# ltatzel/PyTorchHessianFree

Hardware: AMD Instinct MI355X
Metric: GGN-matvecs/sec (damped operator calls inside the PCG loop) (higher is better)
Workload: dtype f32

## Files before the change

### pytorchhessianfree_amd/csrc/hf_conv.hip

```cpp

#include <hip/hip_runtime.h>
#include <stdint.h>
#include <stdlib.h>
#include <string.h>

#include "hf_pcg.h"
#include "hf_unpack.h"

namespace {

typedef float f32x16 __attribute__((ext_vector_type(16)));

constexpr int CT = 256;
#ifndef HF_CONV_BK
#define HF_CONV_BK 32
#endif
constexpr int MAX_TAPS = 64;
#ifndef HF_CONV_FLAT96
#define HF_CONV_FLAT96 1
#endif
#ifndef HF_DCLASS_NOSPLIT
#define HF_DCLASS_NOSPLIT 1
#endif
#ifndef HF_FLAT96_MIN_WORK
#define HF_FLAT96_MIN_WORK 2048
#endif

template <int WM_, int WN_, int TM_, int TN_, int BK_>
struct Cfg {
  static constexpr int WM = WM_, WN = WN_, TM = TM_, TN = TN_, BK = BK_;
  static constexpr int BM = 32 * WM * TM, BN = 32 * WN * TN;
  static constexpr int SM = (BM + 63) / 64 * 64, SN = (BN + 63) / 64 * 64;
  static constexpr int KQ = BK / 4;
  static constexpr int RPT = CT / KQ;
  static constexpr int HK = BK / 2;
  static constexpr int LDK = BK + 4;
  static constexpr int LDA = SM + 4, LDB = SN + 4;
  static constexpr int NT_FLOATS = 2 * (SM + SN) * LDK;
  static constexpr int TN_FLOATS = 2 * BK * (LDA + LDB);
  static constexpr int LDS_FLOATS = (NT_FLOATS > TN_FLOATS ? NT_FLOATS : TN_FLOATS) + 4;
  static_assert(WM * WN == 4, "four waves");
  static_assert(SM / RPT == 2 && SN / RPT == 2, "the hand-counted prefetch ring assumes 2 + 2 loads per step (NT)");
  static_assert(SM == SN, "both operands are staged at the same width");
  static_assert(LDS_FLOATS * 4 <= 64 * 1024, "static LDS limit");
};
typedef Cfg<2, 2, 1, 1, HF_CONV_BK> Small;
typedef Cfg<2, 2, 2, 2, 16> Big;
typedef Cfg<4, 1, 1, 3, 16> Big96;
typedef Cfg<1, 4, 3, 1, 16> Flat96;

struct FastDiv {
  unsigned mul, shift;
};
__host__ __device__ __forceinline__ unsigned fdiv(unsigned n, FastDiv f) {
#if defined(__HIP_DEVICE_COMPILE__)
  return (__umulhi(n, f.mul) + n) >> f.shift;
#else
  return (unsigned)((((unsigned long long)n * f.mul) >> 32) + n) >> f.shift;
#endif
}

struct ConvArgs {
  const float* src;
  const float* mat;
  float* out;
  float* ws;
  int* tickets;
  int dgrad;
  int rows;
  int rh, rw;
  int sh_, sw_;
  int cs, cs_ld;
  int mat_ld;
  int nout, ldc;
  int kout;
  int R, S, stride_h, stride_w, pad_h, pad_w;
  int ntaps;
  int tap_rs[MAX_TAPS];
  int tiles_m, tiles_n, splits, steps;
  int scalar;
  int shift_h, shift_w;
  int out_c;
  int slabs;
  long long slab_stride;
  int big;
  int ncls;
  int cls_tile0[5];
  int cls_tap0[5];
  int cls_h[4], cls_w[4], cls_py[4], cls_px[4];
  FastDiv fd_tiles_n, fd_tiles_m, fd_splits, fd_rw, fd_rh, fd_csteps, fd_cblocks, fd_cs;
  const float *bn_x, *bn_mean, *bn_rstd;
  float *bn_part_x, *bn_part_1;
};

__device__ __forceinline__ void touch_args(const ConvArgs& a) {
  const int* ka = reinterpret_cast<const int*>(&a);
  int sink = 0;
#pragma unroll
  for (unsigned l = 0; l < (sizeof(ConvArgs) + 63) / 64; ++l) {
    const unsigned w = l * 16 < sizeof(ConvArgs) / 4 ? l * 16 : (unsigned)(sizeof(ConvArgs) / 4 - 1);
    sink ^= ka[w];
  }
  asm volatile("" ::"s"(sink));
}

__device__ __forceinline__ int gather_pixel(const ConvArgs& a, int n, int y, int x, int r, int q, bool& valid) {
  int sy, sx;
  bool v = true;
  if (!a.dgrad) {
    sy = y * a.stride_h - a.pad_h + r;
    sx = x * a.stride_w - a.pad_w + q;
  } else {
    const int ty = y + a.pad_h - r, tx = x + a.pad_w - q;
    if (a.shift_h >= 0) { sy = ty >> a.shift_h; sx = tx >> a.shift_w; }
    else { sy = ty / a.stride_h; sx = tx / a.stride_w; }
    v = (ty >= 0) & (tx >= 0) & (sy * a.stride_h == ty) & (sx * a.stride_w == tx);
  }
  v = v & ((unsigned)sy < (unsigned)a.sh_) & ((unsigned)sx < (unsigned)a.sw_);
  valid = v;
  return v ? (n * a.sh_ + sy) * a.sw_ + sx : 0;
}

__device__ __forceinline__ float4 ldg4(const float* p) { return *reinterpret_cast<const float4*>(p); }

typedef float f32x4 __attribute__((ext_vector_type(4)));
__device__ __forceinline__ void gload4(f32x4& dst, const float* p) {
  asm volatile("global_load_dwordx4 %0, %1, off" : "=v"(dst) : "v"(p) : "memory");
}
#define HF_WAIT_SLOT(N, A, B) \
  asm volatile("s_waitcnt vmcnt(" #N ")" : "+v"(A[0]), "+v"(A[1]), "+v"(B[0]), "+v"(B[1]) : : "memory")

__device__ __forceinline__ float4 ldg4s(const float* p, int valid) {
  float4 v = make_float4(0.f, 0.f, 0.f, 0.f);
  if (valid > 0) v.x = p[0];
  if (valid > 1) v.y = p[1];
  if (valid > 2) v.z = p[2];
  if (valid > 3) v.w = p[3];
  return v;
}

template <typename C, bool CLS = false, bool BNSUM = false>
__device__ __forceinline__ void finish_tile(const ConvArgs& a, const f32x16 (&acc)[C::TM][C::TN], int tile, int split,
                                            int wm, int wn, int lane, float* out_tile_base,
                                            int row0, int col0, int row_lim, int col_lim, int ldc,
                                            int* flag_lds, int cls = -1, float* lds = nullptr) {
  constexpr int BM = C::BM, BN = C::BN;
  const int i = lane & 31, h = lane >> 5;
  if constexpr (BNSUM) {
    static_assert(C::TM == 1 && C::TN == 1 && !CLS, "per-tile column sums: 64x64 tiles, plain row enumeration");
    const int col = wn * 32 + i, gcol = col0 + col;
    const bool cok = gcol < col_lim;
    const float mu = cok ? a.bn_mean[gcol] : 0.f, rs = cok ? a.bn_rstd[gcol] : 0.f;
    float xv[16];
#pragma unroll
    for (int reg = 0; reg < 16; ++reg) {
      const int orow = row0 + wm * 32 + (reg & 3) + 8 * (reg >> 2) + 4 * h;
      xv[reg] = (cok && orow < row_lim) ? a.bn_x[(size_t)orow * ldc + gcol] : mu;
    }
    double s1 = 0.0, sx = 0.0;
#pragma unroll
    for (int reg = 0; reg < 16; ++reg) {
      const int orow = row0 + wm * 32 + (reg & 3) + 8 * (reg >> 2) + 4 * h;
      if (cok && orow < row_lim) {
        const float v = acc[0][0][reg];
        s1 += (double)v;
        sx += (double)v * (double)(float)((xv[reg] - mu) * rs);
      }
    }
    double* red = reinterpret_cast<double*>(lds);
    red[(0 * 4 + wm * 2 + h) * BN + col] = s1;
    red[(1 * 4 + wm * 2 + h) * BN + col] = sx;
    __syncthreads();
    const int t = threadIdx.x;
    if (t < 2 * BN) {
      const int kind = t / BN, c = t - kind * BN;
      const double sum = ((red[(kind * 4 + 0) * BN + c] + red[(kind * 4 + 1) * BN + c]) +
                          red[(kind * 4 + 2) * BN + c]) + red[(kind * 4 + 3) * BN + c];
      const int tile_m = (int)fdiv((unsigned)tile, a.fd_tiles_n);
      if (col0 + c < col_lim)
        (kind ? a.bn_part_x : a.bn_part_1)[(size_t)(tile_m * a.splits + split) * a.nout + col0 + c] = (float)sum;
    }
  }
  if (a.splits == 1 || a.slabs) {
    float* dst = out_tile_base + (a.slabs ? (size_t)split * (size_t)a.slab_stride : 0);
#pragma unroll
    for (int im = 0; im < C::TM; ++im)
#pragma unroll
      for (int reg = 0; reg < 16; ++reg) {
        const int row = (wm * C::TM + im) * 32 + (reg & 3) + 8 * (reg >> 2) + 4 * h;
        int orow = row0 + row;
        bool rok = orow < row_lim;
        if (CLS && cls >= 0) {
          const int wc = a.cls_w[cls], hc = a.cls_h[cls];
          const int xq = orow % wc, tq = orow / wc;
          const int yq = tq % hc, nq = tq / hc;
          orow = (nq * a.rh + yq * a.stride_h + a.cls_py[cls]) * a.rw + xq * a.stride_w + a.cls_px[cls];
        }
#pragma unroll
        for (int in = 0; in < C::TN; ++in) {
          const int col = (wn * C::TN + in) * 32 + i;
          if (rok && col0 + col < col_lim) dst[(size_t)orow * ldc + col0 + col] = acc[im][in][reg];
        }
      }
    return;
  }
  const int tiles = a.tiles_m * a.tiles_n;
  float* mine = a.ws + ((size_t)split * tiles + tile) * (BM * BN);
#pragma unroll
  for (int im = 0; im < C::TM; ++im)
#pragma unroll
    for (int in = 0; in < C::TN; ++in)
#pragma unroll
      for (int reg = 0; reg < 16; ++reg) {
        const int row = (wm * C::TM + im) * 32 + (reg & 3) + 8 * (reg >> 2) + 4 * h;
        const int col = (wn * C::TN + in) * 32 + i;
        __hip_atomic_store(mine + row * BN + col, acc[im][in][reg], __ATOMIC_RELAXED, __HIP_MEMORY_SCOPE_AGENT);
      }
  asm volatile("s_waitcnt vmcnt(0)" ::: "memory");
  __syncthreads();
  if (threadIdx.x == 0) {
    const int old = __hip_atomic_fetch_add(a.tickets + tile, 1, __ATOMIC_RELAXED, __HIP_MEMORY_SCOPE_AGENT);
    const int last = old == a.splits - 1;
    if (last) {
      __hip_atomic_store(a.tickets + tile, 0, __ATOMIC_RELAXED, __HIP_MEMORY_SCOPE_AGENT);
      __builtin_amdgcn_fence(__ATOMIC_ACQUIRE, "agent");
      asm volatile("s_waitcnt vmcnt(0)" ::: "memory");
    }
    *flag_lds = last;
  }
  __syncthreads();
  if (!*flag_lds) return;
  const float* base = a.ws + (size_t)tile * (BM * BN);
  const size_t slab = (size_t)tiles * (BM * BN);
  for (int e = threadIdx.x; e < BM * BN / 4; e += CT) {
    float4 s = *reinterpret_cast<const float4*>(base + 4 * e);
    int sp = 1;
    for (; sp + 4 <= a.splits; sp += 4) {
      float4 v[4];
#pragma unroll
      for (int u = 0; u < 4; ++u) v[u] = *reinterpret_cast<const float4*>(base + (sp + u) * slab + 4 * e);
#pragma unroll
      for (int u = 0; u < 4; ++u) { s.x += v[u].x; s.y += v[u].y; s.z += v[u].z; s.w += v[u].w; }
    }
    for (; sp < a.splits; ++sp) {
      const float4 v = *reinterpret_cast<const float4*>(base + sp * slab + 4 * e);
      s.x += v.x; s.y += v.y; s.z += v.z; s.w += v.w;
    }
    const int row = (4 * e) / BN, col = (4 * e) % BN;
    if (row0 + row < row_lim) {
      float* o = out_tile_base + (size_t)(row0 + row) * ldc + col0 + col;
      const float v[4] = {s.x, s.y, s.z, s.w};
#pragma unroll
      for (int c = 0; c < 4; ++c)
        if (col0 + col + c < col_lim) o[c] = v[c];
    }
  }
}

template <bool SCALAR, typename C, bool CLS = false, bool BNSUM = false>
__device__ __forceinline__ void conv_nt_body(const ConvArgs& a, float* lds, int bid) {
  constexpr int BM = C::BM, BN = C::BN, BK = C::BK, KQ = C::KQ, RPT = C::RPT, HK = C::HK, LDK = C::LDK;
  constexpr int NU = 2;
  constexpr int SM = C::SM, SN = C::SN;
  float (*As)[SM][LDK] = reinterpret_cast<float (*)[SM][LDK]>(lds);
  float (*Bs)[SN][LDK] = reinterpret_cast<float (*)[SN][LDK]>(lds + 2 * SM * LDK);
  int& flag = *reinterpret_cast<int*>(lds + C::LDS_FLOATS - 4);
  touch_args(a);
  const int t = threadIdx.x, lane = t & 63, wave = t >> 6, wm = wave / C::WN, wn = wave % C::WN;
  const int bq = (int)fdiv((unsigned)bid, a.fd_tiles_n), tile_n = bid - bq * a.tiles_n;
  const int split = (int)fdiv((unsigned)bq, a.fd_tiles_m), tile_m = bq - split * a.tiles_m;
  const int tile = tile_m * a.tiles_n + tile_n;
  const int csteps = (a.cs + BK - 1) / BK;
  int cls = -1, row_base = tile_m * BM, rows_c = a.rows, tap0 = 0, steps = a.steps;
  if (CLS && a.ncls > 0) {
    cls = 0;
    while (cls + 1 < a.ncls && tile_m >= a.cls_tile0[cls + 1]) ++cls;
    row_base = (tile_m - a.cls_tile0[cls]) * BM;
    rows_c = (a.rows / (a.rh * a.rw)) * a.cls_h[cls] * a.cls_w[cls];
    tap0 = a.cls_tap0[cls];
    steps = (a.cls_tap0[cls + 1] - tap0) * csteps;
  }
  const int per = (int)fdiv((unsigned)(steps + a.splits - 1), a.fd_splits);
  const int j0 = split * per < steps ? split * per : steps, j1 = (j0 + per < steps) ? j0 + per : steps;

  const int lr = t / KQ, kq = t % KQ;
  int rn[NU], ry[NU], rx[NU];
#pragma unroll
  for (int u = 0; u < NU; ++u) {
    const int m = row_base + lr + RPT * u;
    if (m < rows_c) {
      if (CLS && cls >= 0) {
        const int wc = a.cls_w[cls], hc = a.cls_h[cls];
        const int xx = m % wc, tq = m / wc;
        rx[u] = xx * a.stride_w + a.cls_px[cls]; ry[u] = (tq % hc) * a.stride_h + a.cls_py[cls]; rn[u] = tq / hc;
      } else {
        const int tq = (int)fdiv((unsigned)m, a.fd_rw), xx = m - tq * a.rw;
        rn[u] = (int)fdiv((unsigned)tq, a.fd_rh);
        rx[u] = xx; ry[u] = tq - rn[u] * a.rh;
      }
    } else {
      rn[u] = -1; ry[u] = rx[u] = 0;
    }
  }
  const int RS = a.R * a.S;
  const float* brow[NU];
  bool bok[NU];
#pragma unroll
  for (int u = 0; u < NU; ++u) {
    const int j = tile_n * BN + lr + RPT * u;
    bok[u] = (j < a.nout) & (lr + RPT * u < BN);
    brow[u] = a.mat + (size_t)(bok[u] ? j : 0) * RS * a.mat_ld;
  }

  auto fetch = [&](int step, float4 (&ra)[NU], float4 (&rb)[NU]) -> unsigned {
    const int tl = step / csteps, c = (step - tl * csteps) * BK + 4 * kq, ti = tap0 + tl;
    const int rs_ = a.tap_rs[ti], r = rs_ & 255, q = rs_ >> 8;
    const bool cok = c < a.cs;
    unsigned ok = 0;
#pragma unroll
    for (int u = 0; u < NU; ++u) {
      bool va;
      const int pix = gather_pixel(a, rn[u], ry[u], rx[u], r, q, va);
      va = va & cok & (rn[u] >= 0);
      const bool vb = cok & bok[u];
      const float* pa = a.src + (va ? (size_t)pix * a.cs_ld + c : 0);
      const float* pb = vb ? brow[u] + (size_t)(r * a.S + q) * a.mat_ld + c : a.mat;
      ra[u] = ldg4s(pa, va ? a.cs - c : 0);
      rb[u] = ldg4s(pb, vb ? a.cs - c : 0);
      ok |= (va ? 1u : 0u) << (2 * u) | (vb ? 2u : 0u) << (2 * u);
    }
    return ok;
  };
  auto stash = [&](int buf, const float4 (&ra)[NU], const float4 (&rb)[NU], unsigned ok) {
    const float4 zero = make_float4(0.f, 0.f, 0.f, 0.f);
#pragma unroll
    for (int u = 0; u < NU; ++u) {
      *reinterpret_cast<float4*>(&As[buf][lr + RPT * u][4 * kq]) = (ok >> (2 * u)) & 1u ? ra[u] : zero;
      *reinterpret_cast<float4*>(&Bs[buf][lr + RPT * u][4 * kq]) = (ok >> (2 * u)) & 2u ? rb[u] : zero;
    }
  };

  f32x16 acc[C::TM][C::TN];
#pragma unroll
  for (int im = 0; im < C::TM; ++im)
#pragma unroll
    for (int in = 0; in < C::TN; ++in)
#pragma unroll
      for (int r = 0; r < 16; ++r) acc[im][in][r] = 0.f;
  const int i = lane & 31, h = lane >> 5;
  auto compute = [&](int cur) {
    float av[C::TM][HK], bv[C::TN][HK];
#pragma unroll
    for (int im = 0; im < C::TM; ++im) {
      const float* ap = &As[cur][(wm * C::TM + im) * 32 + i][HK * h];
#pragma unroll
      for (int v = 0; v < HK / 4; ++v)
        *reinterpret_cast<float4*>(av[im] + 4 * v) = *reinterpret_cast<const float4*>(ap + 4 * v);
    }
#pragma unroll
    for (int in = 0; in < C::TN; ++in) {
      const float* bp = &Bs[cur][(wn * C::TN + in) * 32 + i][HK * h];
#pragma unroll
      for (int v = 0; v < HK / 4; ++v)
        *reinterpret_cast<float4*>(bv[in] + 4 * v) = *reinterpret_cast<const float4*>(bp + 4 * v);
    }
#pragma unroll
    for (int s = 0; s < HK; ++s)
#pragma unroll
      for (int im = 0; im < C::TM; ++im)
#pragma unroll
        for (int in = 0; in < C::TN; ++in)
          acc[im][in] = __builtin_amdgcn_mfma_f32_32x32x2f32(av[im][s], bv[in][s], acc[im][in], 0, 0, 0);
  };
  const int jl = j1 - 1;
  int cur = 0;
  if (!SCALAR) {
    int f_step = j0, f_ti = (int)fdiv((unsigned)j0, a.fd_csteps), f_cb = j0 - f_ti * csteps;
    auto tap_at = [&](int ti) { return a.tap_rs[ti < MAX_TAPS ? ti : MAX_TAPS - 1]; };
    int f_rs = tap_at(tap0 + f_ti), f_rs_next = tap_at(tap0 + f_ti + 1);
    auto fetch_v = [&](int step, f32x4 (&ra)[NU], f32x4 (&rb)[NU]) -> unsigned {
      if (step > f_step) {
        f_step = step;
        if (++f_cb == csteps) {
          f_cb = 0;
          ++f_ti;
          f_rs = f_rs_next;
          f_rs_next = tap_at(tap0 + f_ti + 1);
        }
      }
      const int c = f_cb * BK + 4 * kq;
      const int rs_ = f_rs, r = rs_ & 255, q = rs_ >> 8;
      const bool cok = c < a.cs;
      unsigned ok = 0;
#pragma unroll
      for (int u = 0; u < NU; ++u) {
        bool va;
        const int pix = gather_pixel(a, rn[u], ry[u], rx[u], r, q, va);
        va = va & cok & (rn[u] >= 0);
        const bool vb = cok & bok[u];
        gload4(ra[u], a.src + (va ? (size_t)pix * a.cs_ld + c : 0));
        gload4(rb[u], vb ? brow[u] + (size_t)(r * a.S + q) * a.mat_ld + c : a.mat);
        ok |= (va ? 1u : 0u) << (2 * u) | (vb ? 2u : 0u) << (2 * u);
      }
      return ok;
    };
    auto stash_v = [&](int buf, const f32x4 (&ra)[NU], const f32x4 (&rb)[NU], unsigned ok) {
      const f32x4 zero = {0.f, 0.f, 0.f, 0.f};
#pragma unroll
      for (int u = 0; u < NU; ++u) {
        *reinterpret_cast<f32x4*>(&As[buf][lr + RPT * u][4 * kq]) = (ok >> (2 * u)) & 1u ? ra[u] : zero;
        *reinterpret_cast<f32x4*>(&Bs[buf][lr + RPT * u][4 * kq]) = (ok >> (2 * u)) & 2u ? rb[u] : zero;
      }
    };
    f32x4 a0[NU], b0[NU], a1[NU], b1[NU], a2[NU], b2[NU];
    unsigned k0 = 0, k1 = 0, k2 = 0;
    if (j0 < j1) {
      k0 = fetch_v(j0, a0, b0);
      k1 = fetch_v(j0 + 1 < j1 ? j0 + 1 : jl, a1, b1);
      k2 = fetch_v(j0 + 2 < j1 ? j0 + 2 : jl, a2, b2);
      for (int j = j0; j < j1; j += 3) {
        HF_WAIT_SLOT(8, a0, b0);
        stash_v(cur, a0, b0, k0);
        __syncthreads();
        k0 = fetch_v(j + 3 < j1 ? j + 3 : jl, a0, b0);
        compute(cur);
        cur ^= 1;
        HF_WAIT_SLOT(8, a1, b1);
        if (j + 1 < j1) {
          stash_v(cur, a1, b1, k1);
          __syncthreads();
          compute(cur);
          cur ^= 1;
        }
        k1 = fetch_v(j + 4 < j1 ? j + 4 : jl, a1, b1);
        HF_WAIT_SLOT(8, a2, b2);
        if (j + 2 < j1) {
          stash_v(cur, a2, b2, k2);
          __syncthreads();
          compute(cur);
          cur ^= 1;
        }
        k2 = fetch_v(j + 5 < j1 ? j + 5 : jl, a2, b2);
      }
      HF_WAIT_SLOT(0, a0, b0);
      HF_WAIT_SLOT(0, a1, b1);
      HF_WAIT_SLOT(0, a2, b2);
    }
  } else {
    float4 a0[NU], b0[NU];
    for (int j = j0; j < j1; ++j) {
      const unsigned k0 = fetch(j, a0, b0);
      stash(cur, a0, b0, k0);
      __syncthreads();
      compute(cur);
      cur ^= 1;
    }
  }
  __syncthreads();
  finish_tile<C, CLS, BNSUM>(a, acc, tile, split, wm, wn, lane, a.out, row_base, tile_n * BN, rows_c, a.nout, a.ldc,
                             &flag, cls, lds);
}

template <bool SCALAR, typename C, bool FLAT = false>
__device__ __forceinline__ void conv_tn_body(const ConvArgs& a, float* lds, int bid) {
  constexpr int BM = C::BM, BN = C::BN, BK = C::BK, HK = C::HK, LDA = C::LDA, LDB = C::LDB;
  float (*As)[BK][LDA] = reinterpret_cast<float (*)[BK][LDA]>(lds);
  float (*Bs)[BK][LDB] = reinterpret_cast<float (*)[BK][LDB]>(lds + 2 * BK * LDA);
  int& flag = *reinterpret_cast<int*>(lds + C::LDS_FLOATS - 4);
  touch_args(a);
  const int t = threadIdx.x, lane = t & 63, wave = t >> 6, wm = wave / C::WN, wn = wave % C::WN;
  const int bq = (int)fdiv((unsigned)bid, a.fd_tiles_n), tile_n = bid - bq * a.tiles_n;
  const int split = (int)fdiv((unsigned)bq, a.fd_tiles_m), tile_m = bq - split * a.tiles_m;
  const int tile = tile_m * a.tiles_n + tile_n;
  const int per = (int)fdiv((unsigned)(a.steps + a.splits - 1), a.fd_splits);
  const int j0 = split * per, j1 = (j0 + per < a.steps) ? j0 + per : a.steps;

  const int cblocks = (a.cs + BN - 1) / BN;
  int ti, c0;
  if constexpr (FLAT) { ti = 0; c0 = tile_n * BN; }
  else { ti = (int)fdiv((unsigned)tile_n, a.fd_cblocks); c0 = (tile_n - ti * cblocks) * BN; }

  constexpr int CQ = C::SM / 4;
  constexpr int RP = CT / CQ;
  constexpr int TU = BK / RP;
  static_assert(TU == 2, "the hand-counted prefetch ring assumes 2 + 2 loads per step (TN)");
  const int kr = t / CQ, cq = t % CQ;
  const int ka = tile_m * BM + 4 * cq;
  int cb = c0 + 4 * cq;
  bool bkok = (cb < a.cs) & (4 * cq < BN);
  if constexpr (FLAT) {
    const int jq = c0 + 4 * cq;
    bkok = (jq < a.ntaps * a.cs) & (4 * cq < BN);
    ti = bkok ? (int)fdiv((unsigned)jq, a.fd_cs) : 0;
    cb = jq - ti * a.cs;
  }
  const int rs_ = a.tap_rs[ti], r = rs_ & 255, q = rs_ >> 8;
  const bool aok = (ka < a.kout) & (4 * cq < BM);

  auto fetch = [&](int step, float4 (&ra)[TU], float4 (&rb)[TU]) -> unsigned {
    unsigned ok = 0;
#pragma unroll
    for (int u = 0; u < TU; ++u) {
      const int m = step * BK + kr + RP * u;
      const bool mok = m < a.rows;
      const int mm = mok ? m : 0;
      const int xx = mm % a.rw, tq = mm / a.rw;
      bool vb;
      const int pix = gather_pixel(a, tq / a.rh, tq % a.rh, xx, r, q, vb);
      vb = vb & mok & bkok;
      const bool va = mok & aok;
      const float* pa = a.mat + (va ? (size_t)m * a.kout + ka : 0);
      const float* pb = a.src + (vb ? (size_t)pix * a.cs_ld + cb : 0);
      ra[u] = ldg4s(pa, va ? a.kout - ka : 0);
      rb[u] = ldg4s(pb, vb ? a.cs - cb : 0);
      ok |= (va ? 1u : 0u) << (2 * u) | (vb ? 2u : 0u) << (2 * u);
    }
    return ok;
  };
  auto stash = [&](int buf, const float4 (&ra)[TU], const float4 (&rb)[TU], unsigned ok) {
    const float4 zero = make_float4(0.f, 0.f, 0.f, 0.f);
#pragma unroll
    for (int u = 0; u < TU; ++u) {
      *reinterpret_cast<float4*>(&As[buf][kr + RP * u][4 * cq]) = (ok >> (2 * u)) & 1u ? ra[u] : zero;
      *reinterpret_cast<float4*>(&Bs[buf][kr + RP * u][4 * cq]) = (ok >> (2 * u)) & 2u ? rb[u] : zero;
    }
  };

  f32x16 acc[C::TM][C::TN];
#pragma unroll
  for (int im = 0; im < C::TM; ++im)
#pragma unroll
    for (int in = 0; in < C::TN; ++in)
#pragma unroll
      for (int x = 0; x < 16; ++x) acc[im][in][x] = 0.f;
  const int i = lane & 31, h = lane >> 5;
  auto compute = [&](int cur) {
    float av[C::TM][HK], bv[C::TN][HK];
#pragma unroll
    for (int s = 0; s < HK; ++s) {
#pragma unroll
      for (int im = 0; im < C::TM; ++im) av[im][s] = As[cur][HK * h + s][(wm * C::TM + im) * 32 + i];
#pragma unroll
      for (int in = 0; in < C::TN; ++in) bv[in][s] = Bs[cur][HK * h + s][(wn * C::TN + in) * 32 + i];
    }
#pragma unroll
    for (int s = 0; s < HK; ++s)
#pragma unroll
      for (int im = 0; im < C::TM; ++im)
#pragma unroll
        for (int in = 0; in < C::TN; ++in)
          acc[im][in] = __builtin_amdgcn_mfma_f32_32x32x2f32(av[im][s], bv[in][s], acc[im][in], 0, 0, 0);
  };
  const int jl = j1 - 1;
  int cur = 0;
  if (!SCALAR) {
    int f_step = j0, fn_[TU], fy_[TU], fx_[TU];
#pragma unroll
    for (int u = 0; u < TU; ++u) {
      const int m = j0 * BK + kr + RP * u;
      const int tq = (int)fdiv((unsigned)m, a.fd_rw), xx = m - tq * a.rw;
      fn_[u] = (int)fdiv((unsigned)tq, a.fd_rh);
      fx_[u] = xx; fy_[u] = tq - fn_[u] * a.rh;
    }
    auto fetch_v = [&](int step, f32x4 (&ra)[TU], f32x4 (&rb)[TU]) -> unsigned {
      if (step > f_step) {
        f_step = step;
#pragma unroll
        for (int u = 0; u < TU; ++u) {
          fx_[u] += BK;
          while (fx_[u] >= a.rw) { fx_[u] -= a.rw; if (++fy_[u] == a.rh) { fy_[u] = 0; ++fn_[u]; } }
        }
      }
      unsigned ok = 0;
#pragma unroll
      for (int u = 0; u < TU; ++u) {
        const int m = step * BK + kr + RP * u;
        const bool mok = m < a.rows;
        bool vb;
        const int pix = gather_pixel(a, fn_[u], fy_[u], fx_[u], r, q, vb);
        vb = vb & mok & bkok;
        const bool va = mok & aok;
        gload4(ra[u], a.mat + (va ? (size_t)m * a.kout + ka : 0));
        gload4(rb[u], a.src + (vb ? (size_t)pix * a.cs_ld + cb : 0));
        ok |= (va ? 1u : 0u) << (2 * u) | (vb ? 2u : 0u) << (2 * u);
      }
      return ok;
    };
    auto stash_v = [&](int buf, const f32x4 (&ra)[TU], const f32x4 (&rb)[TU], unsigned ok) {
      const f32x4 zero = {0.f, 0.f, 0.f, 0.f};
#pragma unroll
      for (int u = 0; u < TU; ++u) {
        *reinterpret_cast<f32x4*>(&As[buf][kr + RP * u][4 * cq]) = (ok >> (2 * u)) & 1u ? ra[u] : zero;
        *reinterpret_cast<f32x4*>(&Bs[buf][kr + RP * u][4 * cq]) = (ok >> (2 * u)) & 2u ? rb[u] : zero;
      }
    };
    f32x4 a0[TU], b0[TU], a1[TU], b1[TU], a2[TU], b2[TU];
    unsigned k0 = 0, k1 = 0, k2 = 0;
    if (j0 < j1) {
      k0 = fetch_v(j0, a0, b0);
      k1 = fetch_v(j0 + 1 < j1 ? j0 + 1 : jl, a1, b1);
      k2 = fetch_v(j0 + 2 < j1 ? j0 + 2 : jl, a2, b2);
      for (int j = j0; j < j1; j += 3) {
        HF_WAIT_SLOT(8, a0, b0);
        stash_v(cur, a0, b0, k0);
        __syncthreads();
        k0 = fetch_v(j + 3 < j1 ? j + 3 : jl, a0, b0);
        compute(cur);
        cur ^= 1;
        HF_WAIT_SLOT(8, a1, b1);
        if (j + 1 < j1) {
          stash_v(cur, a1, b1, k1);
          __syncthreads();
          compute(cur);
          cur ^= 1;
        }
        k1 = fetch_v(j + 4 < j1 ? j + 4 : jl, a1, b1);
        HF_WAIT_SLOT(8, a2, b2);
        if (j + 2 < j1) {
          stash_v(cur, a2, b2, k2);
          __syncthreads();
          compute(cur);
          cur ^= 1;
        }
        k2 = fetch_v(j + 5 < j1 ? j + 5 : jl, a2, b2);
      }
      HF_WAIT_SLOT(0, a0, b0);
      HF_WAIT_SLOT(0, a1, b1);
      HF_WAIT_SLOT(0, a2, b2);
    }
  } else {
    float4 a0[TU], b0[TU];
    for (int j = j0; j < j1; ++j) {
      const unsigned k0 = fetch(j, a0, b0);
      stash(cur, a0, b0, k0);
      __syncthreads();
      compute(cur);
      cur ^= 1;
    }
  }
  __syncthreads();
  if constexpr (FLAT) {
    finish_tile<C>(a, acc, tile, split, wm, wn, lane, a.out, tile_m * BM, c0, a.kout,
                   a.ntaps == 1 ? a.out_c : a.ntaps * a.cs, a.R * a.S * a.out_c, &flag);
  } else {
    float* base = a.out + (size_t)(r * a.S + q) * a.out_c;
    finish_tile<C>(a, acc, tile, split, wm, wn, lane, base, tile_m * BM, c0, a.kout, a.out_c,
                   a.R * a.S * a.out_c, &flag);
  }
}

template <bool SCALAR, typename C, bool CLS = false, bool BNSUM = false>
__global__ __launch_bounds__(CT) void k_conv_nt(const ConvArgs a) {
  __shared__ __attribute__((aligned(16))) float lds[C::LDS_FLOATS];
  conv_nt_body<SCALAR, C, CLS, BNSUM>(a, lds, blockIdx.x);
}

template <bool SCALAR, typename C>
__global__ __launch_bounds__(CT) void k_conv_nt_unpack(const ConvArgs a, const hf_shared::UnpackArgs u,
                                                       const float* __restrict__ usrc, int conv_blocks) {
  __shared__ __attribute__((aligned(16))) float lds[C::LDS_FLOATS];
  if ((int)blockIdx.x < conv_blocks) conv_nt_body<SCALAR, C, false>(a, lds, blockIdx.x);
  else hf_shared::unpack_block<float>(usrc, u, blockIdx.x - (unsigned)conv_blocks);
}

template <bool SCALAR, typename C, bool FLAT = false>
__global__ __launch_bounds__(CT) void k_conv_tn(const ConvArgs a) {
  __shared__ __attribute__((aligned(16))) float lds[C::LDS_FLOATS];
  conv_tn_body<SCALAR, C, FLAT>(a, lds, blockIdx.x);
}

template <bool ANYBIG, bool CLS = false>
__global__ __launch_bounds__(CT) void k_conv_dw(const ConvArgs d, const ConvArgs w, int nblocks_d) {
  constexpr int LDSB = Big::LDS_FLOATS > Big96::LDS_FLOATS ? Big::LDS_FLOATS : Big96::LDS_FLOATS;
  constexpr int LDSF = ANYBIG ? (LDSB > Small::LDS_FLOATS ? LDSB : Small::LDS_FLOATS) : Small::LDS_FLOATS;
  __shared__ __attribute__((aligned(16))) float lds[LDSF];
  if ((int)blockIdx.x < nblocks_d) {
    if (ANYBIG && d.big == 1) conv_nt_body<false, Big, CLS>(d, lds, blockIdx.x);
    else if (ANYBIG && d.big == 2) conv_nt_body<false, Big96, CLS>(d, lds, blockIdx.x);
    else conv_nt_body<false, Small, CLS>(d, lds, blockIdx.x);
  } else {
    if (ANYBIG && w.big == 1) conv_tn_body<false, Big>(w, lds, blockIdx.x - nblocks_d);
    else if (ANYBIG && w.big == 2) conv_tn_body<false, Big96>(w, lds, blockIdx.x - nblocks_d);
    else if (ANYBIG && w.big == 3) conv_tn_body<false, Flat96, true>(w, lds, blockIdx.x - nblocks_d);
    else conv_tn_body<false, Small>(w, lds, blockIdx.x - nblocks_d);
  }
}

constexpr int GROUP_MAX = 4;
struct GroupMeta {
  int tn[GROUP_MAX];
  int start[GROUP_MAX + 1];
  int n;
};

template <bool ANYBIG, bool CLS, bool BNSUM = false>
__device__ __forceinline__ void group_run(const ConvArgs& a, int tn, float* lds, int local) {
  if constexpr (BNSUM) {
    if (a.bn_part_1) conv_nt_body<false, Small, false, true>(a, lds, local);
    else conv_nt_body<false, Small, false, false>(a, lds, local);
    return;
  }
  if (tn) {
    if (ANYBIG && a.big == 1) conv_tn_body<false, Big>(a, lds, local);
    else if (ANYBIG && a.big == 2) conv_tn_body<false, Big96>(a, lds, local);
    else if (ANYBIG && a.big == 3) conv_tn_body<false, Flat96, true>(a, lds, local);
    else conv_tn_body<false, Small>(a, lds, local);
  } else {
    if (ANYBIG && a.big == 1) conv_nt_body<false, Big, CLS>(a, lds, local);
    else if (ANYBIG && a.big == 2) conv_nt_body<false, Big96, CLS>(a, lds, local);
    else conv_nt_body<false, Small, CLS>(a, lds, local);
  }
}

template <bool ANYBIG, bool CLS = false, bool BNSUM = false>
__global__ __launch_bounds__(CT) void k_conv_group(const ConvArgs a0, const ConvArgs a1, const ConvArgs a2,
                                                   const ConvArgs a3, const GroupMeta m) {
  constexpr int LDSB = Big::LDS_FLOATS > Big96::LDS_FLOATS ? Big::LDS_FLOATS : Big96::LDS_FLOATS;
  constexpr int LDSF = ANYBIG ? (LDSB > Small::LDS_FLOATS ? LDSB : Small::LDS_FLOATS) : Small::LDS_FLOATS;
  __shared__ __attribute__((aligned(16))) float lds[LDSF];
  const int b = (int)blockIdx.x;
  if (b < m.start[1]) group_run<ANYBIG, CLS, BNSUM>(a0, m.tn[0], lds, b);
  else if (b < m.start[2]) group_run<ANYBIG, CLS, BNSUM>(a1, m.tn[1], lds, b - m.start[1]);
  else if (b < m.start[3]) group_run<ANYBIG, CLS, BNSUM>(a2, m.tn[2], lds, b - m.start[2]);
  else group_run<ANYBIG, CLS, BNSUM>(a3, m.tn[3], lds, b - m.start[3]);
}

inline bool aligned16(const void* p) { return (((uintptr_t)p) & 15) == 0; }

}

#define HF_HIP(expr)                         \
  do {                                       \
    hipError_t e_ = (expr);                  \
    if (e_ != hipSuccess) return (int)e_;    \
  } while (0)

namespace {

#ifndef HF_BIG_TARGET_BLOCKS
#define HF_BIG_TARGET_BLOCKS 512
#endif
#ifndef HF_BIG_MIN_WORK
#define HF_BIG_MIN_WORK 6144
#endif
constexpr int64_t BIG_TARGET_BLOCKS = HF_BIG_TARGET_BLOCKS;
constexpr int64_t FEW_TILES = 8;
constexpr int64_t FEW_TILES_CAP = 96;

int choose_splits(int64_t tiles, int64_t steps, int target_blocks, int64_t ws_bytes, bool slabs = false,
                  int bk = Small::BK, int64_t tile_elems = Small::BM * Small::BN) {
  int64_t best = 1;
  if (slabs && target_blocks <= 0) {
    const bool big = bk != Small::BK;
    best = ((big ? BIG_TARGET_BLOCKS : 256) + tiles - 1) / tiles;
    if (big && best > steps / 8) best = steps / 8;
    if (best > steps / 2) best = steps / 2;
    const int64_t cap = tiles <= FEW_TILES ? FEW_TILES_CAP : (big ? 128 : 32);
    if (best > cap) best = cap;
    if (best < 1) best = 1;
    while (best > 1 && ((steps + best - 1) / best) * (best - 1) >= steps) --best;
    return (int)best;
  }
  if (target_blocks > 0) {
    best = (target_blocks + tiles - 1) / tiles;
    if (best > steps / 2) best = steps / 2;
    if (best < 1) best = 1;
  } else {
    double best_cost = 1e30;
    const int64_t cap = steps < 64 ? steps : 64;
    for (int64_t sp = 1; sp <= cap; ++sp) {
      const int64_t per = (steps + sp - 1) / sp;
      if (sp > 1 && per * (sp - 1) >= steps) continue;
      const double rounds = (double)(tiles * sp) / 512.0;
      double cost = (0.6 + 0.014 * bk) * (double)per * (rounds > 1.0 ? rounds : 1.0);
      if (sp > 1) cost += 3.0 + 0.15 * (double)sp;
      if (cost < best_cost - 1e-9) { best_cost = cost; best = sp; }
    }
  }
  while (!slabs && best > 1 && best * tiles * tile_elems * (int64_t)sizeof(float) > ws_bytes) --best;
  while (best > 1 && ((steps + best - 1) / best) * (best - 1) >= steps) --best;
  return (int)best;
}

FastDiv make_fastdiv(int64_t d) {
  if (d < 1) d = 1;
  unsigned l = 0;
  while ((1LL << l) < d) ++l;
  FastDiv f;
  f.mul = (unsigned)((((unsigned long long)((1ULL << l) - (unsigned long long)d)) << 32) / (unsigned long long)d + 1);
  f.shift = l;
  return f;
}

void seal(ConvArgs& a) {
  const int bk = a.big ? Big::BK : Small::BK;
  const int bn = a.big == 1 ? Big::BN : a.big == 2 ? Big96::BN : Small::BN;
  a.fd_tiles_n = make_fastdiv(a.tiles_n);
  a.fd_tiles_m = make_fastdiv(a.tiles_m);
  a.fd_splits = make_fastdiv(a.splits);
  a.fd_rw = make_fastdiv(a.rw);
  a.fd_rh = make_fastdiv(a.rh);
  a.fd_csteps = make_fastdiv((a.cs + bk - 1) / bk);
  a.fd_cblocks = make_fastdiv((a.cs + bn - 1) / bn);
  a.fd_cs = make_fastdiv(a.cs);
}

void launch_one(int direction, const ConvArgs& a_in, int64_t blocks, hipStream_t stream) {
  ConvArgs a = a_in;
  seal(a);
  const dim3 grid((unsigned)blocks), block(CT);
  if (direction <= 1) {
    if (a.scalar) hipLaunchKernelGGL((k_conv_nt<true, Small>), grid, block, 0, stream, a);
    else if (a.ncls > 0 && a.big == 1) hipLaunchKernelGGL((k_conv_nt<false, Big, true>), grid, block, 0, stream, a);
    else if (a.ncls > 0 && a.big == 2) hipLaunchKernelGGL((k_conv_nt<false, Big96, true>), grid, block, 0, stream, a);
    else if (a.ncls > 0) hipLaunchKernelGGL((k_conv_nt<false, Small, true>), grid, block, 0, stream, a);
    else if (a.big == 1) hipLaunchKernelGGL((k_conv_nt<false, Big>), grid, block, 0, stream, a);
    else if (a.big == 2) hipLaunchKernelGGL((k_conv_nt<false, Big96>), grid, block, 0, stream, a);
    else hipLaunchKernelGGL((k_conv_nt<false, Small>), grid, block, 0, stream, a);
  } else {
    if (a.scalar) hipLaunchKernelGGL((k_conv_tn<true, Small>), grid, block, 0, stream, a);
    else if (a.big == 1) hipLaunchKernelGGL((k_conv_tn<false, Big>), grid, block, 0, stream, a);
    else if (a.big == 2) hipLaunchKernelGGL((k_conv_tn<false, Big96>), grid, block, 0, stream, a);
    else if (a.big == 3) hipLaunchKernelGGL((k_conv_tn<false, Flat96, true>), grid, block, 0, stream, a);
    else hipLaunchKernelGGL((k_conv_tn<false, Small>), grid, block, 0, stream, a);
  }
}

void launch_dw(const ConvArgs& d_in, const ConvArgs& w_in, int64_t bd, int64_t bw, hipStream_t stream) {
  ConvArgs d = d_in, w = w_in;
  seal(d);
  seal(w);
  const dim3 grid((unsigned)(bd + bw)), block(CT);
  const bool big = d.big || w.big, cls = d.ncls > 0;
  if (big && cls) hipLaunchKernelGGL((k_conv_dw<true, true>), grid, block, 0, stream, d, w, (int)bd);
  else if (big) hipLaunchKernelGGL((k_conv_dw<true, false>), grid, block, 0, stream, d, w, (int)bd);
  else if (cls) hipLaunchKernelGGL((k_conv_dw<false, true>), grid, block, 0, stream, d, w, (int)bd);
  else hipLaunchKernelGGL((k_conv_dw<false, false>), grid, block, 0, stream, d, w, (int)bd);
}

void launch_unpack(const ConvArgs& a_in, int64_t blocks, const hf_shared::UnpackArgs& u, const float* usrc,
                   int ublocks, hipStream_t stream) {
  ConvArgs a = a_in;
  seal(a);
  const dim3 grid((unsigned)(blocks + ublocks)), block(CT);
  if (a.scalar) hipLaunchKernelGGL((k_conv_nt_unpack<true, Small>), grid, block, 0, stream, a, u, usrc, (int)blocks);
  else hipLaunchKernelGGL((k_conv_nt_unpack<false, Small>), grid, block, 0, stream, a, u, usrc, (int)blocks);
}

int group_add(GroupMeta& m, int i, bool tn, int64_t blocks) {
  const int64_t end = m.start[i] + blocks;
  if (end > 0x7fffffffLL) return HF_ERR_ARG;
  m.tn[i] = tn;
  for (int j = i + 1; j <= GROUP_MAX; ++j) m.start[j] = (int)end;
  m.n = i + 1;
  return HF_OK;
}

void launch_group(ConvArgs (&a)[GROUP_MAX], const GroupMeta& m, bool bnsum, hipStream_t st) {
  bool big = false, cls = false;
  for (int i = 0; i < m.n; ++i) {
    big = big || a[i].big;
    cls = cls || a[i].ncls > 0;
    seal(a[i]);
  }
  const dim3 grid((unsigned)m.start[GROUP_MAX]), block(CT);
  if (bnsum && m.n == 1 && a[0].bn_part_1)
    hipLaunchKernelGGL((k_conv_nt<false, Small, false, true>), grid, block, 0, st, a[0]);
  else if (bnsum) hipLaunchKernelGGL((k_conv_group<false, false, true>), grid, block, 0, st, a[0], a[1], a[2], a[3], m);
  else if (big && cls) hipLaunchKernelGGL((k_conv_group<true, true>), grid, block, 0, st, a[0], a[1], a[2], a[3], m);
  else if (big) hipLaunchKernelGGL((k_conv_group<true, false>), grid, block, 0, st, a[0], a[1], a[2], a[3], m);
  else if (cls) hipLaunchKernelGGL((k_conv_group<false, true>), grid, block, 0, st, a[0], a[1], a[2], a[3], m);
  else hipLaunchKernelGGL((k_conv_group<false, false>), grid, block, 0, st, a[0], a[1], a[2], a[3], m);
}

int want_big(int direction, int64_t rows, int64_t dim_m, int64_t dim_n, int64_t red, int64_t mult, bool scalar,
             bool all_taps = false, bool slab_mode = false) {
  if (scalar) return 0;
  auto fill = [](int64_t d, int64_t t) { return (double)d / (double)(((d + t - 1) / t) * t); };
  const double f128 = fill(dim_m, 128) * fill(dim_n, 128), f96 = fill(dim_m, 128) * fill(dim_n, 96);
  int kind = f96 > f128 + 1e-9 ? 2 : 1;
  double fbest = kind == 2 ? f96 : f128;
  int64_t flat_tiles = 0;
  if (HF_CONV_FLAT96 && direction == 2 && all_taps && dim_m % 96 == 0 && dim_n % 4 == 0) {
    const double fflat = fill(mult * dim_n, 128);
    if (fflat > fbest + 0.05) { kind = 3; fbest = fflat; flat_tiles = (dim_m / 96) * ((mult * dim_n + 127) / 128); }
  }
  const bool fits = fbest >= 0.7;
  const int64_t tiles = kind == 3 ? flat_tiles
                                  : ((dim_m + 127) / 128) * ((dim_n + (kind == 2 ? 95 : 127)) / (kind == 2 ? 96 : 128)) * mult;
  const int64_t steps = (red + Big::BK - 1) / Big::BK;
  const int64_t least = (kind == 3 && slab_mode) ? HF_FLAT96_MIN_WORK : HF_BIG_MIN_WORK;
  return (fits && rows >= 2048 && tiles * steps >= least) ? kind : 0;
}

static int apply_out_c(ConvArgs& a, int64_t out_c) {
  if (!out_c) return HF_OK;
  if (a.big == 3 && out_c != a.cs && a.ntaps != 1) return HF_ERR_ARG;
  a.out_c = (int)out_c;
  return HF_OK;
}

struct Scratch {
  float* ws;
  int64_t ws_bytes;
  int* tickets;
  int64_t n_tickets;
  int target_blocks;
};

int64_t setup(ConvArgs& a, const hf_conv_problem& p, const Scratch* sc, bool tickets) {
  const int direction = p.direction, slab_splits = tickets ? -1 : p.splits, target_blocks = sc ? sc->target_blocks : 0;
  const int64_t n = p.n, h = p.h, w = p.w, c = p.c, k = p.k, r = p.r, s = p.s, stride_h = p.stride_h,
                stride_w = p.stride_w, pad_h = p.pad_h, pad_w = p.pad_w;
  const int64_t oh = (h + 2 * pad_h - r) / stride_h + 1, ow = (w + 2 * pad_w - s) / stride_w + 1;
  memset(&a, 0, sizeof(a));
  a.src = (const float*)p.act;
  a.mat = (const float*)p.mat;
  a.out = (float*)p.out;
  a.ws = sc ? sc->ws : nullptr;
  a.tickets = sc ? sc->tickets : nullptr;
  a.R = (int)r; a.S = (int)s;
  a.stride_h = (int)stride_h; a.stride_w = (int)stride_w; a.pad_h = (int)pad_h; a.pad_w = (int)pad_w;
  a.shift_h = a.shift_w = -1;
  if ((stride_h & (stride_h - 1)) == 0 && (stride_w & (stride_w - 1)) == 0) {
    a.shift_h = a.shift_w = 0;
    while ((1 << a.shift_h) < stride_h) ++a.shift_h;
    while ((1 << a.shift_w) < stride_w) ++a.shift_w;
  }
  for (int rr = 0; rr < r; ++rr) {
    bool live_r = false;
    for (int64_t y = 0; y < oh && !live_r; ++y) { const int64_t iy = y * stride_h - pad_h + rr; live_r = iy >= 0 && iy < h; }
    if (!live_r) continue;
    for (int qq = 0; qq < s; ++qq) {
      bool live_q = false;
      for (int64_t x = 0; x < ow && !live_q; ++x) { const int64_t ix = x * stride_w - pad_w + qq; live_q = ix >= 0 && ix < w; }
      if (live_q) { a.tap_rs[a.ntaps] = rr | (qq << 8); a.ntaps++; }
    }
  }
  if (a.ntaps == 0) return HF_ERR_ARG;
  int64_t rows, red_steps;
  if (direction == 0) {
    a.dgrad = 0; rows = n * oh * ow; a.rh = (int)oh; a.rw = (int)ow; a.sh_ = (int)h; a.sw_ = (int)w;
    a.cs = (int)c; a.nout = (int)k; a.ldc = (int)k;
  } else if (direction == 1) {
    a.dgrad = 1; rows = n * h * w; a.rh = (int)h; a.rw = (int)w; a.sh_ = (int)oh; a.sw_ = (int)ow;
    a.cs = (int)k; a.nout = (int)c; a.ldc = (int)c;
  } else {
    a.dgrad = 0; rows = n * oh * ow; a.rh = (int)oh; a.rw = (int)ow; a.sh_ = (int)h; a.sw_ = (int)w;
    a.cs = (int)c; a.kout = (int)k;
  }
  a.out_c = a.cs;
  a.rows = (int)rows;
  a.cs_ld = (int)(p.act_ld > 0 ? p.act_ld : a.cs);
  a.mat_ld = (int)(p.mat_ld > 0 ? p.mat_ld : a.cs);
  a.scalar = ((c % 4) || (k % 4) || (a.cs_ld % 4) || (a.mat_ld % 4)) ? 1 : 0;
  if (a.cs_ld < a.cs || a.mat_ld < a.cs || (p.mat_ld > 0 && direction == 2)) return HF_ERR_ARG;
  int cls_taps_max = a.ntaps;
  const bool classes = direction == 1 && slab_splits >= 0 && (stride_h > 1 || stride_w > 1) &&
                       stride_h * stride_w <= 4 && !a.scalar && n * h * w >= 2048;
  struct { int py, px, hc, wc, ntaps; unsigned char r[MAX_TAPS], q[MAX_TAPS]; } cl[4];
  int ncls = 0;
  if (classes) {
    cls_taps_max = 0;
    for (int py = 0; py < stride_h; ++py)
      for (int px = 0; px < stride_w; ++px) {
        const int hc = (int)((h - py + stride_h - 1) / stride_h), wc = (int)((w - px + stride_w - 1) / stride_w);
        if (hc <= 0 || wc <= 0) continue;
        auto& c_ = cl[ncls];
        c_.py = py; c_.px = px; c_.hc = hc; c_.wc = wc; c_.ntaps = 0;
        for (int t_ = 0; t_ < a.ntaps; ++t_) {
          const int rr = a.tap_rs[t_] & 255, qq = a.tap_rs[t_] >> 8;
          const int64_t dy = py + pad_h - rr, dx = px + pad_w - qq;
          if (((dy % stride_h) + stride_h) % stride_h == 0 && ((dx % stride_w) + stride_w) % stride_w == 0) {
            c_.r[c_.ntaps] = (unsigned char)rr; c_.q[c_.ntaps] = (unsigned char)qq; c_.ntaps++;
          }
        }
        if (c_.ntaps > cls_taps_max) cls_taps_max = c_.ntaps;
        ++ncls;
      }
  }
  a.big = direction <= 1 ? want_big(direction, rows, rows, a.nout, (int64_t)cls_taps_max * a.cs, 1, a.scalar)
                         : want_big(direction, rows, a.kout, a.cs, rows, a.ntaps, a.scalar, a.ntaps == (int)(r * s),
                                    slab_splits >= 0);
  const int BM = a.big == 3 ? Flat96::BM : a.big ? Big::BM : Small::BM;
  const int BN = a.big == 2 ? Big96::BN : a.big ? Big::BN : Small::BN;
  const int BK = a.big ? Big::BK : Small::BK;
  if (direction <= 1) {
    a.tiles_m = (int)((rows + BM - 1) / BM);
    a.tiles_n = (a.nout + BN - 1) / BN;
    red_steps = (int64_t)cls_taps_max * ((a.cs + BK - 1) / BK);
    if (ncls > 0) {
      a.ncls = ncls;
      int tile0 = 0, tap0 = 0;
      for (int i = 0; i < ncls; ++i) {
        a.cls_tile0[i] = tile0; a.cls_tap0[i] = tap0;
        a.cls_h[i] = cl[i].hc; a.cls_w[i] = cl[i].wc; a.cls_py[i] = cl[i].py; a.cls_px[i] = cl[i].px;
        for (int t_ = 0; t_ < cl[i].ntaps; ++t_) a.tap_rs[tap0 + t_] = cl[i].r[t_] | (cl[i].q[t_] << 8);
        tap0 += cl[i].ntaps;
        tile0 += (int)((n * cl[i].hc * cl[i].wc + BM - 1) / BM);
      }
      a.cls_tile0[ncls] = tile0; a.cls_tap0[ncls] = tap0;
      a.tiles_m = tile0;
      if (red_steps < 1) red_steps = 1;
    }
  } else {
    a.tiles_m = (a.kout + BM - 1) / BM;
    a.tiles_n = a.big == 3 ? (a.ntaps * a.cs + BN - 1) / BN : a.ntaps * ((a.cs + BN - 1) / BN);
    red_steps = (rows + BK - 1) / BK;
  }
// ... 255 lines not shown
```

Baseline: 1662.

## Add multi-stage load ring with interleaved MFMA schedule for small weight-grad conv tiles

Adds a software-pipelined path for the weight-gradient (TN) convolution body when the tile config is Small with a single MFMA accumulator. Global loads are issued RING steps ahead into a register ring and waited on with precise vmcnt counts. LDS stashes, fragment reads and barriers are interleaved between individual MFMAs using sched_barrier fences. Geometry scalars are pinned to SGPRs and a forward-only gather is used. This aims to hide memory latency behind compute, at the cost of more registers and a hand-fixed schedule; it only applies in kernels instantiated without big tiles.

```diff
diff --git a/pytorchhessianfree_amd/csrc/hf_conv.hip b/pytorchhessianfree_amd/csrc/hf_conv.hip
--- a/pytorchhessianfree_amd/csrc/hf_conv.hip
+++ b/pytorchhessianfree_amd/csrc/hf_conv.hip
@@ -121,6 +121,23 @@
   return v ? (n * a.sh_ + sy) * a.sw_ + sx : 0;
 }
 
+struct Geom {
+  int sth, stw, ph, pw, sh, sw;
+};
+__device__ __forceinline__ void pin(int& v) { asm volatile("" : "+s"(v)); }
+__device__ __forceinline__ void pin(unsigned& v) { asm volatile("" : "+s"(v)); }
+__device__ __forceinline__ Geom make_geom(const ConvArgs& a) {
+  Geom g = {a.stride_h, a.stride_w, a.pad_h, a.pad_w, a.sh_, a.sw_};
+  pin(g.sth); pin(g.stw); pin(g.ph); pin(g.pw); pin(g.sh); pin(g.sw);
+  return g;
+}
+__device__ __forceinline__ int gather_pixel_fwd(const Geom& g, int n, int y, int x, int r, int q, bool& valid) {
+  const int sy = y * g.sth - g.ph + r, sx = x * g.stw - g.pw + q;
+  const bool v = ((unsigned)sy < (unsigned)g.sh) & ((unsigned)sx < (unsigned)g.sw);
+  valid = v;
+  return v ? (n * g.sh + sy) * g.sw + sx : 0;
+}
+
 __device__ __forceinline__ float4 ldg4(const float* p) { return *reinterpret_cast<const float4*>(p); }
 
 typedef float f32x4 __attribute__((ext_vector_type(4)));
@@ -129,6 +146,103 @@
 }
 #define HF_WAIT_SLOT(N, A, B) \
   asm volatile("s_waitcnt vmcnt(" #N ")" : "+v"(A[0]), "+v"(A[1]), "+v"(B[0]), "+v"(B[1]) : : "memory")
+
+#ifndef HF_CONV_RING
+#define HF_CONV_RING 2
+#endif
+constexpr int RING = HF_CONV_RING;
+#define HF_WAIT_RING(A, B)                                                              \
+  asm volatile("s_waitcnt vmcnt(%[n])" : "+v"(A[0]), "+v"(A[1]), "+v"(B[0]), "+v"(B[1]) \
+               : [n] "n"(4 * (RING - 1)) : "memory")
+#define HF_DRAIN_RING(A, B) \
+  asm volatile("s_waitcnt vmcnt(0)" : "+v"(A[0]), "+v"(A[1]), "+v"(B[0]), "+v"(B[1]) : : "memory")
+
+template <typename Prep, typename Load, typename Stash, typename Frag>
+__device__ __forceinline__ void pipelined_share(int j0, int j1, f32x16& acc, Prep&& prep, Load&& load, Stash&& stash,
+                                                Frag&& frag) {
+  static_assert(RING % 2 == 0 && RING >= 2 && RING <= 14,
+                "LDS buffer and fragment set of a step are compile-time in the unrolled ring; vmcnt counts to 63");
+  f32x4 ra[RING][2], rb[RING][2];
+  unsigned ok[RING];
+  float av[2][16], bv[2][16];
+  if (j0 >= j1) return;
+#pragma unroll
+  for (int s = 0; s < RING; ++s) {
+    prep(j0 + s < j1);
+    ok[s] = load(0, ra[s][0]);
+    ok[s] |= load(1, rb[s][0]);
+    ok[s] |= load(2, ra[s][1]);
+    ok[s] |= load(3, rb[s][1]);
+  }
+  HF_WAIT_RING(ra[0], rb[0]);
+  stash(0, 0, ra[0][0], rb[0][0], ok[0]);
+  stash(0, 1, ra[0][1], rb[0][1], ok[0]);
+  prep(j0 + RING < j1);
+  ok[0] = load(0, ra[0][0]);
+  ok[0] |= load(1, rb[0][0]);
+  ok[0] |= load(2, ra[0][1]);
+  ok[0] |= load(3, rb[0][1]);
+  __syncthreads();
+#pragma unroll
+  for (int piece = 0; piece < 4; ++piece) frag(0, piece, av[0], bv[0]);
+#define HF_STEP_MFMA(K) acc = __builtin_amdgcn_mfma_f32_32x32x2f32(av[p][K], bv[p][K], acc, 0, 0, 0)
+#define HF_SCHED_FENCE __builtin_amdgcn_sched_barrier(0)
+  for (int j = j0; j < j1; j += RING) {
+#pragma unroll
+    for (int s = 0; s < RING; ++s) {
+      if (j + s >= j1) break;
+      const int p = s & 1, q = p ^ 1, n = (s + 1) % RING;
+      HF_SCHED_FENCE;
+      HF_STEP_MFMA(0);
+      HF_WAIT_RING(ra[n], rb[n]);
+      HF_SCHED_FENCE;
+      HF_STEP_MFMA(1);
+      stash(q, 0, ra[n][0], rb[n][0], ok[n]);
+      HF_SCHED_FENCE;
+      HF_STEP_MFMA(2);
+      stash(q, 1, ra[n][1], rb[n][1], ok[n]);
+      HF_SCHED_FENCE;
+      HF_STEP_MFMA(3);
+      prep(j + s + 1 + RING < j1);
+      unsigned k = load(0, ra[n][0]);
+      HF_SCHED_FENCE;
+      HF_STEP_MFMA(4);
+      k |= load(1, rb[n][0]);
+      HF_SCHED_FENCE;
+      HF_STEP_MFMA(5);
+      k |= load(2, ra[n][1]);
+      HF_SCHED_FENCE;
+      HF_STEP_MFMA(6);
+      k |= load(3, rb[n][1]);
+      ok[n] = k;
+      HF_SCHED_FENCE;
+      HF_STEP_MFMA(7);
+      __syncthreads();
+      HF_SCHED_FENCE;
+      HF_STEP_MFMA(8);
+      frag(q, 0, av[q], bv[q]);
+      HF_SCHED_FENCE;
+      HF_STEP_MFMA(9);
+      frag(q, 1, av[q], bv[q]);
+      HF_SCHED_FENCE;
+      HF_STEP_MFMA(10);
+      frag(q, 2, av[q], bv[q]);
+      HF_SCHED_FENCE;
+      HF_STEP_MFMA(11);
+      frag(q, 3, av[q], bv[q]);
+      HF_SCHED_FENCE;
+      HF_STEP_MFMA(12);
+      HF_STEP_MFMA(13);
+      HF_STEP_MFMA(14);
+      HF_STEP_MFMA(15);
+      HF_SCHED_FENCE;
+    }
+  }
+#undef HF_STEP_MFMA
+#undef HF_SCHED_FENCE
+#pragma unroll
+  for (int s = 0; s < RING; ++s) HF_DRAIN_RING(ra[s], rb[s]);
+}
 
 __device__ __forceinline__ float4 ldg4s(const float* p, int valid) {
   float4 v = make_float4(0.f, 0.f, 0.f, 0.f);
@@ -461,7 +575,7 @@
                              &flag, cls, lds);
 }
 
-template <bool SCALAR, typename C, bool FLAT = false>
+template <bool SCALAR, typename C, bool FLAT = false, bool PIPE = true>
 __device__ __forceinline__ void conv_tn_body(const ConvArgs& a, float* lds, int bid) {
   constexpr int BM = C::BM, BN = C::BN, BK = C::BK, HK = C::HK, LDA = C::LDA, LDB = C::LDB;
   float (*As)[BK][LDA] = reinterpret_cast<float (*)[BK][LDA]>(lds);
@@ -553,7 +667,55 @@
   };
   const int jl = j1 - 1;
   int cur = 0;
-  if (!SCALAR) {
+  if constexpr (!SCALAR && PIPE && C::TM * C::TN == 1 && !FLAT) {
+    const Geom g = make_geom(a);
+    int g_rows = a.rows, g_kout = a.kout, g_cs_ld = a.cs_ld, g_rw = a.rw, g_rh = a.rh;
+    pin(g_rows); pin(g_kout); pin(g_cs_ld); pin(g_rw); pin(g_rh);
+    FastDiv g_frw = a.fd_rw, g_frh = a.fd_rh;
+    pin(g_frw.mul); pin(g_frw.shift); pin(g_frh.mul); pin(g_frh.shift);
+    const float *g_src = a.src, *g_mat = a.mat;
+    int f_m0 = j0 * BK + kr;
+    int p_m0 = 0;
+    bool p_live = false;
+    auto prep = [&](bool live) {
+      p_m0 = f_m0;
+      p_live = live;
+      f_m0 += BK;
+    };
+    auto load = [&](int piece, f32x4& dst) -> unsigned {
+      const int u = piece >> 1;
+      const int m = p_m0 + RP * u;
+      const bool mok = (m < g_rows) & p_live;
+      if (!(piece & 1)) {
+        const bool va = mok & aok;
+        gload4(dst, g_mat + (va ? (size_t)m * g_kout + ka : 0));
+        return (va ? 1u : 0u) << (2 * u);
+      }
+      const int mm = mok ? m : 0;
+      const int tq = (int)fdiv((unsigned)mm, g_frw), xx = mm - tq * g_rw;
+      const int nn = (int)fdiv((unsigned)tq, g_frh), yy = tq - nn * g_rh;
+      bool vb;
+      const int pix = gather_pixel_fwd(g, nn, yy, xx, r, q, vb);
+      vb = vb & mok & bkok;
+      gload4(dst, g_src + (vb ? (size_t)pix * g_cs_ld + cb : 0));
+      return (vb ? 2u : 0u) << (2 * u);
+    };
+    auto stash_u = [&](int buf, int u, const f32x4& ra, const f32x4& rb, unsigned ok) {
+      const f32x4 zero = {0.f, 0.f, 0.f, 0.f};
+      *reinterpret_cast<f32x4*>(&As[buf][kr + RP * u][4 * cq]) = (ok >> (2 * u)) & 1u ? ra : zero;
+      *reinterpret_cast<f32x4*>(&Bs[buf][kr + RP * u][4 * cq]) = (ok >> (2 * u)) & 2u ? rb : zero;
+    };
+    auto frag = [&](int buf, int piece, float (&av)[HK], float (&bv)[HK]) {
+      static_assert(HK == 16, "four fragment pieces of eight elements each");
+      const int s0 = 8 * (piece & 1);
+#pragma unroll
+      for (int s = s0; s < s0 + 8; ++s) {
+        if (piece < 2) av[s] = As[buf][HK * h + s][wm * 32 + i];
+        else bv[s] = Bs[buf][HK * h + s][wn * 32 + i];
+      }
+    };
+    pipelined_share(j0, j1, acc[0][0], prep, load, stash_u, frag);
+  } else if (!SCALAR) {
     int f_step = j0, fn_[TU], fy_[TU], fx_[TU];
 #pragma unroll
     for (int u = 0; u < TU; ++u) {
@@ -682,7 +844,7 @@
     if (ANYBIG && w.big == 1) conv_tn_body<false, Big>(w, lds, blockIdx.x - nblocks_d);
     else if (ANYBIG && w.big == 2) conv_tn_body<false, Big96>(w, lds, blockIdx.x - nblocks_d);
     else if (ANYBIG && w.big == 3) conv_tn_body<false, Flat96, true>(w, lds, blockIdx.x - nblocks_d);
-    else conv_tn_body<false, Small>(w, lds, blockIdx.x - nblocks_d);
+    else conv_tn_body<false, Small, false, !ANYBIG>(w, lds, blockIdx.x - nblocks_d);
   }
 }
 
@@ -704,7 +866,7 @@
     if (ANYBIG && a.big == 1) conv_tn_body<false, Big>(a, lds, local);
     else if (ANYBIG && a.big == 2) conv_tn_body<false, Big96>(a, lds, local);
     else if (ANYBIG && a.big == 3) conv_tn_body<false, Flat96, true>(a, lds, local);
-    else conv_tn_body<false, Small>(a, lds, local);
+    else conv_tn_body<false, Small, false, !ANYBIG>(a, lds, local);
   } else {
     if (ANYBIG && a.big == 1) conv_nt_body<false, Big, CLS>(a, lds, local);
     else if (ANYBIG && a.big == 2) conv_nt_body<false, Big96, CLS>(a, lds, local);
```

Result: faster. 1717, median of 6 (+3.3%).
